# sevagh/xumx-sliCQ

Hardware: AMD Instinct MI355X
Metric: real-time factor (audio-s demixed / wall-s), 44.1 kHz stereo, offline model (higher is better)
Workload: dtype f32; 1 GPU; BASELINE configs[1]: offline model (Bark-262 sliCQT), one 240 s stereo track (10,584,000 samples, 5 chunks) per GPU, Wiener off (mix-phase), seeded synthetic weights; parallelism=one track per rank, 1 rank(s), no data-path collective

## Files before the change

xumx_slicq_amd/csrc/cdae.hip:

```cpp
#include <algorithm>
#include <cmath>
#include <cstdlib>
#include <cstring>
#include <vector>

#include "../../include/xumx_slicq_hip.h"
#include "gemm_tile.h"
#include "gemm_tile_bf3.h"
#include "gemm_tile_bf6.h"
#include "plan.h"
#include "prof.h"

#include "cdae_api.h"

namespace xsq {

__global__ __launch_bounds__(256) void k_magnitude_whiten(const float4* __restrict__ X, float4* __restrict__ xin,
                                                           const int64_t* __restrict__ cum,
                                                           const CdaeBlockDev* __restrict__ blocks,
                                                           const float* __restrict__ mean,
                                                           const float* __restrict__ scale, int nblocks,
                                                           int BC, int S, int64_t nquads, int split) {
    __shared__ int64_t cum_s[128];
    for (int i = threadIdx.x; i < nblocks && i < 128; i += 256) cum_s[i] = cum[i];
// ... 290 lines not shown
        g.in = a.act3 + (int64_t)CS * a.Bn * a.T1 * (4 * (int64_t)b.cumF1 + (int64_t)tgt * b.F1);
        g.out = nullptr;
        return g;
    }
    __device__ RowA row_a(const Group& g, int m) const {
        RowA r; r.p = nullptr; r.f = 0; r.t = 0; r.vo = BUF_OOB;
        if (m >= g.M) return r;
        int b, f, t;
        split_row(m, g.Fo, g.To, b, f, t);
        r.f = f; r.t = t;
        r.p = g.in + (((int64_t)b * g.Fi + f) * g.Ti + t) * CS;
        r.vo = 4u * (unsigned)(((b * g.Fi + f) * g.Ti + t) * CS);
        return r;
    }
    struct Cursor { int k, kk, df; };
    __device__ Cursor cursor(const Group& g, int k) const {
        Cursor c;
        c.k = k; c.df = k / (2 * CS); c.kk = k - c.df * 2 * CS;
        return c;
    }
    __device__ void advance(const Group& g, Cursor& c) const {
        c.k += 16; c.kk += 16;
        if (c.kk >= 2 * CS) { c.kk -= 2 * CS; ++c.df; }
    }
    __device__ float4 load_a4(const Group& g, const RowA& r, const Cursor& c) const { return load_at(g, r, c.k, c.df, c.kk); }
    __device__ float4 load_a4(const Group& g, const RowA& r, int k) const {
        const int df = k / (2 * CS);
        return load_at(g, r, k, df, k - df * 2 * CS);
    }
    __device__ float4 load_at(const Group& g, const RowA& r, int k, int df, int kk) const {
        const int fi = r.f - df;
        const bool pos_ok = kk < CS ? r.t >= 1 : r.t < g.Ti;
        const bool ok = k < g.K && (unsigned)fi < (unsigned)g.Fi && pos_ok;
        const unsigned vo = r.vo + 4u * (unsigned)(kk - (df * g.Ti + 1) * CS);
        return buf_ld4(buf_rsrc(g.in, 0x40000000u), ok ? vo : BUF_OOB, 0);
    }
    __device__ void epilogue(const Group& g, int row0, int n, const f32x16& a0, const f32x16& a1, bool wide) const {
        const bool v0 = n < g.N, v1 = wide && n + 32 < g.N;
        const int n1 = n + 32;
        const int ca = n >= g.hop, cb = n1 >= g.hop;
        const int dta = n - ca * g.hop, dtb = n1 - cb * g.hop;
        if (a.gx8) {
            const int64_t STp = (int64_t)g.To * g.hop, FSTp = (int64_t)g.F * STp;
            float* o = a.gx8 + 4 * (int64_t)a.Bn * g.To * g.cum + (int64_t)g.tgt * a.Bn * 2 * FSTp;
            int b, f, u;
            split_row(row0, g.Fo, g.To, b, f, u);
            int prev = 0;
#pragma unroll
            for (int r = 0; r < 16; ++r) {
                u += acc_row(r) - prev; prev = acc_row(r);
                while (u >= g.To) { u -= g.To; if (++f == g.Fo) { f = 0; ++b; } }
                if (row0 + acc_row(r) >= g.M) break;
                float* d = o + (int64_t)(b * 2) * FSTp + (int64_t)f * STp + (int64_t)u * g.hop;
                if (v0) d[ca * FSTp + dta] = a0[r];
                if (v1) d[cb * FSTp + dtb] = a1[r];
            }
            return;
        }
        const float ba = g.shift[ca], bb = g.shift[cb];
        const int FST = g.F * a.S * g.T;
        const int perb = g.Fo * g.To;
        const float2* X2 = reinterpret_cast<const float2*>(a.X) + (int64_t)a.Bn * 2 * a.S * g.cum;
        float2* Y2 = reinterpret_cast<float2*>(a.Y) + (int64_t)a.Bn * 8 * a.S * g.cum + (int64_t)g.tgt * a.Bn * 2 * FST;
        float* Mk = a.masks ? a.masks + (int64_t)a.Bn * 8 * a.S * g.cum + (int64_t)g.tgt * a.Bn * 2 * FST : nullptr;
        const int offa = ca * FST + dta, offb = cb * FST + dtb;
        const int slab0 = row0 & ~31;
        const int b0 = slab0 / perb;
        const int next_b = (b0 + 1) * perb;
        if (slab0 + 32 <= g.M && perb >= 32) {
            const int obase = row0 * g.hop + b0 * FST, ocut = next_b - row0;
            auto off = [&](int r) { return obase + acc_row(r) * g.hop + (acc_row(r) >= ocut ? FST : 0); };
            if (!a.Y && next_b >= slab0 + 32) {
                const int s0 = __builtin_amdgcn_readfirstlane(slab0);
                const int b0u = __builtin_amdgcn_readfirstlane(b0);
                const __amdgpu_buffer_rsrc_t rm = buf_rsrc(Mk + (int64_t)s0 * g.hop + (int64_t)b0u * FST, 0x40000000u);
                const unsigned lane_off = 4u * (unsigned)((row0 - slab0) * g.hop);
                const unsigned va = v0 ? lane_off + 4u * (unsigned)offa : BUF_OOB, vb = v1 ? lane_off + 4u * (unsigned)offb : BUF_OOB;
#pragma unroll
                for (int r = 0; r < 16; ++r)
                    __builtin_amdgcn_raw_buffer_store_b32(__builtin_bit_cast(unsigned, __builtin_amdgcn_rcpf(1.f + __expf(-(a0[r] + ba)))), rm, (int)va, 4 * acc_row(r) * g.hop, 0);
                if (wide) {
#pragma unroll
                    for (int r = 0; r < 16; ++r)
                        __builtin_amdgcn_raw_buffer_store_b32(__builtin_bit_cast(unsigned, __builtin_amdgcn_rcpf(1.f + __expf(-(a1[r] + bb)))), rm, (int)vb, 4 * acc_row(r) * g.hop, 0);
                }
                return;
            }
            if (!a.Y) {
                if (v0) {
#pragma unroll
                    for (int r = 0; r < 16; ++r) Mk[off(r) + offa] = __builtin_amdgcn_rcpf(1.f + __expf(-(a0[r] + ba)));
                }
                if (v1) {
#pragma unroll
                    for (int r = 0; r < 16; ++r) Mk[off(r) + offb] = __builtin_amdgcn_rcpf(1.f + __expf(-(a1[r] + bb)));
                }
                return;
            }
#pragma unroll
            for (int r0 = 0; r0 < 16; r0 += 4) {
                if (v0) {
                    float2 x[4];
#pragma unroll
                    for (int q = 0; q < 4; ++q) x[q] = X2[off(r0 + q) + offa];
#pragma unroll
                    for (int q = 0; q < 4; ++q) {
                        const float mk = __builtin_amdgcn_rcpf(1.f + __expf(-(a0[r0 + q] + ba)));
                        Y2[off(r0 + q) + offa] = make_float2(mk * x[q].x, mk * x[q].y);
                    }
                }
                if (v1) {
                    float2 x[4];
#pragma unroll
                    for (int q = 0; q < 4; ++q) x[q] = X2[off(r0 + q) + offb];
#pragma unroll
                    for (int q = 0; q < 4; ++q) {
                        const float mk = __builtin_amdgcn_rcpf(1.f + __expf(-(a1[r0 + q] + bb)));
                        Y2[off(r0 + q) + offb] = make_float2(mk * x[q].x, mk * x[q].y);
                    }
                }
            }
            if (Mk) {
                if (v0) {
#pragma unroll
                    for (int r = 0; r < 16; ++r) Mk[off(r) + offa] = __builtin_amdgcn_rcpf(1.f + __expf(-(a0[r] + ba)));
                }
                if (v1) {
#pragma unroll
                    for (int r = 0; r < 16; ++r) Mk[off(r) + offb] = __builtin_amdgcn_rcpf(1.f + __expf(-(a1[r] + bb)));
                }
            }
            return;
        }
#pragma unroll
        for (int r = 0; r < 16; ++r) {
            const int m = row0 + acc_row(r);
            if (m >= g.M) break;
            const int o = m * g.hop + (m / perb) * FST;
            if (v0) {
                const float mk = __builtin_amdgcn_rcpf(1.f + __expf(-(a0[r] + ba)));
                if (a.Y) { const float2 x = X2[o + offa]; Y2[o + offa] = make_float2(mk * x.x, mk * x.y); }
                if (Mk) Mk[o + offa] = mk;
            }
            if (v1) {
                const float mk = __builtin_amdgcn_rcpf(1.f + __expf(-(a1[r] + bb)));
                if (a.Y) { const float2 x = X2[o + offb]; Y2[o + offb] = make_float2(mk * x.x, mk * x.y); }
                if (Mk) Mk[o + offb] = mk;
            }
        }
    }
    __device__ void epilogue16(const Group& g, int rowb, int lane, int n0, const f32x4 (&acc)[2]) const {
        const int n = n0 + (lane & 15), q16 = lane >> 4;
        if (n >= g.N) return;
        const int c = n >= g.hop, dt = n - c * g.hop;
        const float bias = g.shift[c];
        const int FST = g.F * a.S * g.T, perb = g.Fo * g.To;
        const float2* X2 = reinterpret_cast<const float2*>(a.X) + (int64_t)a.Bn * 2 * a.S * g.cum;
        float2* Y2 = a.Y ? reinterpret_cast<float2*>(a.Y) + (int64_t)a.Bn * 8 * a.S * g.cum + (int64_t)g.tgt * a.Bn * 2 * FST : nullptr;
        float* Mk = a.masks ? a.masks + (int64_t)a.Bn * 8 * a.S * g.cum + (int64_t)g.tgt * a.Bn * 2 * FST : nullptr;
        const int off = c * FST + dt;
        if (!Y2 && rowb + 32 <= g.M && perb >= 32) {
            const int m0 = rowb + 4 * q16;
            const int b0 = rowb / perb;
            const int obase = m0 * g.hop + b0 * FST + off, ocut = (b0 + 1) * perb - m0;
            float mk[2][4];
#pragma unroll
            for (int rb = 0; rb < 2; ++rb)
#pragma unroll
                for (int r = 0; r < 4; ++r) mk[rb][r] = __builtin_amdgcn_rcpf(1.f + __expf(-(acc[rb][r] + bias)));
#pragma unroll
            for (int rb = 0; rb < 2; ++rb)
#pragma unroll
                for (int r = 0; r < 4; ++r) {
                    const int dm = 16 * rb + r;
                    Mk[obase + dm * g.hop + (dm >= ocut ? FST : 0)] = mk[rb][r];
                }
            return;
        }
#pragma unroll
        for (int rb = 0; rb < 2; ++rb)
#pragma unroll
            for (int r = 0; r < 4; ++r) {
                const int m = rowb + 16 * rb + 4 * q16 + r;
                if (m >= g.M) continue;
                const int o = m * g.hop + (m / perb) * FST + off;
                const float mk = __builtin_amdgcn_rcpf(1.f + __expf(-(acc[rb][r] + bias)));
                if (Y2) { const float2 x = X2[o]; Y2[o] = make_float2(mk * x.x, mk * x.y); }
                if (Mk) Mk[o] = mk;
            }
    }
};

}
#include "cdae_slab.h"
#include "cdae_wino.h"
#include "cdae_wino23.h"
#include "cdae_wino4.h"
#include "cdae_l1f.h"
#include "cdae_l4f.h"
namespace xsq {


static bool wino4_wanted() { return getenv("XSQ_WINO4") && atoi(getenv("XSQ_WINO4")) != 0; }

static int kf_of(int F) { return F < 10 ? 1 : (F < 20 ? 3 : 5); }

static int get_cdae_tiles(xsq_model* Mo, int layer, int Bn, int S, TileTable* out, bool n16 = false, bool tgt_outer = false) {
    const TileKey key{TileKind::CdaeGemm, Bn, S, layer, (n16 ? 1 : 0) | (tgt_outer ? 2 : 0)};
    return cached_tiles<TileDev>(Mo->mu, Mo->tiles, key, out, [&](std::vector<TileDev>& t) {
        const int T1 = Mo->causal ? 2 * S : 2 * S - 1, T2 = T1 - 3;
        const std::vector<int> order = order_descending(Mo->nblocks, [&](int b) {
            const CdaeBlockDev& d = Mo->blocks[b];
            return layer == 1 ? 2 * d.kf * d.T : (layer >= 4 ? d.kf * 2 * CS : d.kf * 4 * CS);
        });
        for (int b : order) {
            const CdaeBlockDev& d = Mo->blocks[b];
            int64_t M; int N;
            switch (layer) {
                case 1: M = (int64_t)Bn * d.F1 * T1; N = CS; break;
                case 2: M = (int64_t)Bn * d.F2 * T2; N = CS; break;
                case 3: M = (int64_t)Bn * d.F1 * T1; N = CS; break;
                case 4: M = (int64_t)Bn * d.F * 2 * S; N = d.T; break;
                default: M = (int64_t)Bn * d.F * (T1 + 1); N = d.T; break;
            }
            if (layer == 1 || layer == 4 || layer == 6) {
                auto push = [&](int64_t m0, int n0, int tgt) {
                    const int rem = N - n0;
                    const int kind = n16 ? (rem <= 16 ? 2 : rem <= 32 ? 1 : rem <= 48 ? 3 : 0) : (rem <= 32 ? 1 : 0);
                    t.push_back(TileDev{b * 4 + tgt, (int)m0, n0, kind});
                };
                if (tgt_outer) {
                    for (int tgt = 0; tgt < NT; ++tgt)
                        for (int64_t m0 = 0; m0 < M; m0 += 128)
                            for (int n0 = 0; n0 < N; n0 += 64) push(m0, n0, tgt);
                } else {
                    for (int64_t m0 = 0; m0 < M; m0 += 128)
                        for (int n0 = 0; n0 < N; n0 += 64)
                            for (int tgt = 0; tgt < NT; ++tgt) push(m0, n0, tgt);
                }
            } else {
                for (int tgt = 0; tgt < NT; ++tgt) push_group_tiles(t, b * 4 + tgt, M, N);
            }
        }
    });
}

static std::vector<int> blocks_by_taps(const xsq_model* Mo) {
    return order_descending(Mo->nblocks, [&](int b) { return Mo->blocks[b].kf; });
}

static int get_slab_tiles(xsq_model* Mo, int layer, int Bn, int S, TileTable* out) {
    return cached_tiles<SlabTileDev>(Mo->mu, Mo->tiles, TileKey{TileKind::CdaeSlab, Bn, S, layer, 0}, out, [&](std::vector<SlabTileDev>& t) {
        const int T1 = Mo->causal ? 2 * S : 2 * S - 1, T2 = T1 - 3;
        for (int b : blocks_by_taps(Mo)) {
            const CdaeBlockDev& d = Mo->blocks[b];
            const int64_t perb = layer == 2 ? (int64_t)d.F2 * T2 : (int64_t)d.F1 * T1;
            for (int tgt = 0; tgt < NT; ++tgt) {
                const int64_t off1 = (int64_t)CS * Bn * T1 * (4 * (int64_t)d.cumF1 + (int64_t)tgt * d.F1);
                const int64_t off2 = (int64_t)CS * Bn * T2 * (4 * (int64_t)d.cumF2 + (int64_t)tgt * d.F2);
                SlabTileDev e;
                e.kf = d.kf;
                if (layer == 2) { e.Fo = d.F2; e.Fi = d.F1; e.in_off = off1; e.out_off = off2; e.shift_off = d.s2[tgt]; e.w_off = d.w2[tgt]; }
                else { e.Fo = d.F1; e.Fi = d.F2; e.in_off = off2; e.out_off = off1; e.shift_off = d.s3[tgt]; e.w_off = d.w3[tgt]; }
                const int To = layer == 2 ? T2 : T1;
                e.pad = 0;
                for (int bi = 0; bi < Bn; ++bi)
                    for (int64_t r = 0; r < perb; r += SLAB_ROWS) {
                        e.m0 = (int)(bi * perb + r); e.b = bi; e.f0 = (int)(r / To); e.t0 = (int)(r % To);
                        t.push_back(e);
                    }
            }
        }
    });
}

static bool block_fuses23(const CdaeBlockDev& d) { return d.kf == 1 && d.F1 == d.F2; }

static int get_wino_tiles(xsq_model* Mo, int layer, int Bn, int S, TileTable* out, int outs = 2, bool skip_fused = false) {
    return cached_tiles<WinoTileDev>(Mo->mu, Mo->tiles, TileKey{TileKind::CdaeWino, Bn, S, layer, outs | (skip_fused ? 16 : 0)}, out, [&](std::vector<WinoTileDev>& t) {
        const int T1 = Mo->causal ? 2 * S : 2 * S - 1, T2 = T1 - 3;
        const int To = layer == 2 ? T2 : T1, P = (To + outs - 1) / outs, len = outs == 4 ? W4_QUADS : WN_PAIRS;
        for (int b : blocks_by_taps(Mo)) {
            const CdaeBlockDev& d = Mo->blocks[b];
            if (skip_fused && block_fuses23(d)) continue;
            for (int tgt = 0; tgt < NT; ++tgt) {
                const int64_t off1 = (int64_t)CS * Bn * T1 * (4 * (int64_t)d.cumF1 + (int64_t)tgt * d.F1);
                const int64_t off2 = (int64_t)CS * Bn * T2 * (4 * (int64_t)d.cumF2 + (int64_t)tgt * d.F2);
                WinoTileDev e;
                e.kf = d.kf; e.P = P;
                if (layer == 2) { e.Fo = d.F2; e.Fi = d.F1; e.in_off = off1; e.out_off = off2; e.shift_off = d.s2[tgt]; e.u_off = (outs == 4 ? d.uq2 : d.u2)[tgt]; }
                else { e.Fo = d.F1; e.Fi = d.F2; e.in_off = off2; e.out_off = off1; e.shift_off = d.s3[tgt]; e.u_off = (outs == 4 ? d.uq3 : d.u3)[tgt]; }
                const int perb = e.Fo * P;
                e.pad0 = e.pad1 = 0;
                for (int bi = 0; bi < Bn; ++bi)
                    for (int Q = 0; Q < perb; Q += len) {
                        e.Q0 = Q; e.b = bi;
                        t.push_back(e);
                    }
            }
        }
    });
}

static int get_wino23_tiles(xsq_model* Mo, int Bn, int S, TileTable* out) {
    return cached_tiles<Wino23TileDev>(Mo->mu, Mo->tiles, TileKey{TileKind::CdaeWino23, Bn, S, 23, 0}, out, [&](std::vector<Wino23TileDev>& t) {
        const int T1 = Mo->causal ? 2 * S : 2 * S - 1, P = (T1 + 1) / 2;
        for (int b : blocks_by_taps(Mo)) {
            const CdaeBlockDev& d = Mo->blocks[b];
            if (!block_fuses23(d)) continue;
            for (int tgt = 0; tgt < NT; ++tgt) {
                Wino23TileDev e;
                e.F = d.F1;
                e.in_off = e.out_off = (int64_t)CS * Bn * T1 * (4 * (int64_t)d.cumF1 + (int64_t)tgt * d.F1);
                e.shift2_off = d.s2[tgt]; e.shift3_off = d.s3[tgt]; e.u2_off = d.u2[tgt]; e.u3_off = d.u3[tgt];
                for (int bi = 0; bi < Bn; ++bi)
                    for (int f = 0; f < d.F1; ++f)
                        for (int A = 0; A < P; A += WN23_OUT) {
                            e.A = A; e.f = f; e.b = bi;
                            t.push_back(e);
                        }
            }
        }
    });
}

static int get_l1f_tiles(xsq_model* Mo, int Bn, int S, TileTable* out) {
    return cached_tiles<L1fTileDev>(Mo->mu, Mo->tiles, TileKey{TileKind::CdaeL1f, Bn, S, 1, 0}, out, [&](std::vector<L1fTileDev>& t) {
        const int T1 = 2 * S - 1, P = (T1 + 1) / 2;
        for (int b : order_descending(Mo->nblocks, [&](int b) { return Mo->blocks[b].nch1; })) {
            const CdaeBlockDev& d = Mo->blocks[b];
            L1fTileDev e;
            e.kf = d.kf; e.F = d.F; e.F1 = d.F1; e.hop = d.hop; e.nchunks = d.nch1; e.P = P;
            e.in_off = (int64_t)Bn * 2 * S * d.cum;
            const int total = Bn * d.F1 * P;
            e.pad0 = 0;
            for (int Q = 0; Q < total; Q += LF_PAIRS)
                for (int tgt = 0; tgt < NT; ++tgt) {
                    e.Q0 = Q;
                    e.out_off = (int64_t)CS * Bn * T1 * (4 * (int64_t)d.cumF1 + (int64_t)tgt * d.F1);
                    e.shift_off = d.s1[tgt]; e.u_off = d.u1[tgt];
                    t.push_back(e);
                }
        }
    });
}

static const int L4F_RUN = 6;
static int get_l4f_tiles(xsq_model* Mo, int Bn, int S, TileTable* out) {
    return cached_tiles<L4fTileDev>(Mo->mu, Mo->tiles, TileKey{TileKind::CdaeL4f, Bn, S, 4, 0}, out, [&](std::vector<L4fTileDev>& t) {
        const int T1 = 2 * S - 1, P = S;
        for (int b : blocks_by_taps(Mo)) {
            const CdaeBlockDev& d = Mo->blocks[b];
            const int W = d.T, cols = l4f_cols(W);
            const int64_t FST = (int64_t)d.F * S * d.T;
            L4fTileDev e;
            e.kf = d.kf; e.F = d.F; e.hop = d.hop; e.P = P; e.x_off = (int)((int64_t)Bn * 2 * S * d.cum);
            const int total = Bn * d.F * P;
            const int rtiles = (total + L4_PAIRS - 1) / L4_PAIRS;
            const int nruns = d.kf == 1 ? (rtiles + L4F_RUN - 1) / L4F_RUN : rtiles;
            for (int tgt = 0; tgt < NT; ++tgt) {
                e.in_off = (int64_t)CS * Bn * T1 * (4 * (int64_t)d.cumF1 + (int64_t)tgt * d.F1);
                e.out_off = (int64_t)Bn * 8 * S * d.cum + (int64_t)tgt * Bn * 2 * FST;
                e.bias_off = d.b4[tgt];
                for (int r = 0; r < nruns; ++r) {
                    const int t0 = (int)((int64_t)rtiles * r / nruns), t1 = (int)((int64_t)rtiles * (r + 1) / nruns);
                    for (int n0 = 0; n0 < cols; n0 += 64) {
                        e.Q0 = t0 * L4_PAIRS; e.run = t1 - t0; e.n0 = n0;
                        e.u_off = d.u4[tgt] + (int64_t)3 * CS * n0;
                        t.push_back(e);
                    }
                }
            }
        }
    });
}

}

using namespace xsq;

extern "C" {

int64_t xsq_model_num_params(int nblocks, const int32_t* F, const int32_t* T) {
    if (!F || !T || nblocks <= 0) return XSQ_ERR_ARG;
    int64_t n = 0;
    for (int b = 0; b < nblocks; ++b) {
        const int kf = kf_of(F[b]);
        n += 2 * F[b];
        n += NT * ((int64_t)H1 * 2 * kf * T[b] + 4 * H1 + (int64_t)H2 * H1 * kf * 4 + 4 * H2 +
                   (int64_t)H2 * H1 * kf * 4 + 4 * H1 + (int64_t)H1 * 2 * kf * T[b] + 2);
    }
    return n;
}

static int model_build(xsq_model** out, int nblocks, const int32_t* F, const int32_t* T, int causal,
                       const float* params, int64_t nparams, xsq_model** partial);

int xsq_model_create(xsq_model** out, int nblocks, const int32_t* F, const int32_t* T, int causal,
                     const float* params, int64_t nparams) {
    xsq_model* partial = nullptr;
    const int rc = model_build(out, nblocks, F, T, causal, params, nparams, &partial);
    if (rc != XSQ_OK && partial) xsq_model_destroy(partial);
    return rc;
}

static int model_build(xsq_model** out, int nblocks, const int32_t* F, const int32_t* T, int causal,
                       const float* params, int64_t nparams, xsq_model** partial) {
    XSQ_REQUIRE(out && F && T && params && nblocks > 0, "xsq_model_create: null argument");
    XSQ_REQUIRE(nparams == xsq_model_num_params(nblocks, F, T),
                "xsq_model_create: got %lld parameters, the block table needs %lld", (long long)nparams,
                (long long)xsq_model_num_params(nblocks, F, T));
    std::vector<BlockHost> table;
    int64_t sumFT = 0;
    for (int b = 0; b < nblocks; ++b) {
        XSQ_REQUIRE(F[b] >= 1 && T[b] >= 4 && T[b] % 4 == 0, "xsq_model_create: block %d has F=%d T=%d", b, F[b], T[b]);
        XSQ_REQUIRE(F[b] - 2 * (kf_of(F[b]) - 1) >= 1, "xsq_model_create: block with F=%d too small", F[b]);
        table.push_back(BlockHost{0, F[b], T[b], sumFT});
        sumFT += (int64_t)F[b] * T[b];
    }
    xsq_model* Mo = new xsq_model();
    *partial = Mo;
    Mo->causal = causal ? 1 : 0; Mo->nblocks = nblocks; Mo->sumFT = sumFT; Mo->table = table;
    Mo->wino4 = wino4_wanted();
    std::vector<float> pool, upool, mean, scale;
    std::vector<int64_t> cum(nblocks + 1, 0);
    std::vector<int> blockF(nblocks);
    const float* p = params;
    int cumF1 = 0, cumF2 = 0;
    int64_t cumF = 0;
    auto alloc = [&](size_t n) { size_t o = pool.size(); pool.resize(o + n, 0.f); return (int64_t)o; };
    auto bn_fold = [&](const float* bn, int C, int co, int64_t shift_off) {
        const float *bw = bn, *bb = bn + C, *rm = bn + 2 * C, *rv = bn + 3 * C;
        const double s = (double)bw[co] / std::sqrt((double)rv[co] + 1e-5);
        pool[shift_off + co] = (float)((double)bb[co] - (double)rm[co] * s);
        return s;
    };
    auto wino_weights = [&](const double (*G)[4], int ncomp, int UDF, int (*u_off)(int, int, int), int64_t wsrc, int kf) {
        const int K2 = kf * 4 * CS;
        const int64_t u = (int64_t)upool.size();
        upool.resize(upool.size() + (size_t)kf * UDF, 0.f);
        for (int df = 0; df < kf; ++df)
            for (int j = 0; j < ncomp; ++j)
                for (int col = 0; col < WN_COLS; ++col)
                    for (int ci = 0; ci < CS; ++ci) {
                        double acc = 0.0;
                        for (int dt = 0; dt < 4; ++dt)
                            acc += G[j][dt] * (double)pool[wsrc + (size_t)col * K2 + (df * 4 + dt) * CS + ci];
                        upool[u + (size_t)df * UDF + u_off(j, col, ci)] = (float)acc;
                    }
        return u;
    };
    for (int bi = 0; bi < nblocks; ++bi) {
        const BlockHost& hb = table[bi];
        CdaeBlockDev d;
        memset(&d, 0, sizeof(d));
        d.F = hb.F; d.T = hb.T; d.hop = hb.T / 2; d.kf = kf_of(hb.F);
        d.F1 = d.F - d.kf + 1; d.F2 = d.F1 - d.kf + 1;
        d.cumF1 = cumF1; d.cumF2 = cumF2; d.cum = hb.cum; d.cumF = cumF;
        d.ld1 = (int)round_up(2 * d.kf * d.T, 16); d.ld4 = (int)round_up(d.kf * 2 * CS, 16);
        cumF1 += d.F1; cumF2 += d.F2; cumF += d.F;
        cum[bi] = hb.cum; blockF[bi] = d.F;
        const int kf = d.kf, W = d.T, hop = d.hop;
        mean.insert(mean.end(), p, p + d.F); p += d.F;
        scale.insert(scale.end(), p, p + d.F); p += d.F;
        for (int t = 0; t < NT; ++t) {
            const float* w = p; p += (size_t)H1 * 2 * kf * W;
            const float* bn = p; p += 4 * H1;
            const int K1 = 2 * kf * W;
            d.w1[t] = alloc((size_t)64 * d.ld1);
            d.s1[t] = alloc(64);
            for (int co = 0; co < H1; ++co) {
                const double s = bn_fold(bn, H1, co, d.s1[t]);
                for (int k = 0; k < K1; ++k)
                    pool[d.w1[t] + (size_t)co * d.ld1 + k] = (float)((double)w[(size_t)co * K1 + k] * s);
            }
            {
                d.nch1 = l1f_chunks(kf, hop);
                const int64_t u = (int64_t)upool.size();
                upool.resize(upool.size() + (size_t)d.nch1 * LF_U16, 0.f);
                d.u1[t] = u;
                const int hq = (hop + 3) / 4;
                for (int s = 0; s < d.nch1; ++s)
                    for (int kk = 0; kk < 16; ++kk) {
                        const int e4 = 4 * s + kk / 4, seg = e4 / hq, dd = 4 * (e4 % hq) + kk % 4;
                        if (seg >= 2 * kf || dd >= hop) continue;
                        for (int co = 0; co < H1; ++co) {
                            const double w0 = pool[d.w1[t] + (size_t)co * d.ld1 + (size_t)seg * W + dd];
                            const double w1v = pool[d.w1[t] + (size_t)co * d.ld1 + (size_t)seg * W + hop + dd];
                            upool[u + l1f_u_off(s, 0, co, kk)] = (float)w0;
                            upool[u + l1f_u_off(s, 1, co, kk)] = (float)(w0 + w1v);
                            upool[u + l1f_u_off(s, 2, co, kk)] = (float)w1v;
                        }
                    }
            }
            w = p; p += (size_t)H2 * H1 * kf * 4;
            bn = p; p += 4 * H2;
            const int K2 = kf * 4 * CS;
            d.w2[t] = alloc((size_t)64 * K2);
            d.s2[t] = alloc(64);
            for (int co = 0; co < H2; ++co) {
                const double s = bn_fold(bn, H2, co, d.s2[t]);
                for (int ci = 0; ci < H1; ++ci)
                    for (int df = 0; df < kf; ++df)
                        for (int dt = 0; dt < 4; ++dt)
                            pool[d.w2[t] + (size_t)co * K2 + (df * 4 + dt) * CS + ci] =
                                (float)((double)w[(((size_t)co * H1 + ci) * kf + df) * 4 + dt] * s);
            }
            w = p; p += (size_t)H2 * H1 * kf * 4;
            bn = p; p += 4 * H1;
            d.w3[t] = alloc((size_t)64 * K2);
            d.s3[t] = alloc(64);
            for (int co = 0; co < H1; ++co) {
                const double s = bn_fold(bn, H1, co, d.s3[t]);
                for (int ci = 0; ci < H2; ++ci)
                    for (int df = 0; df < kf; ++df)
                        for (int dt = 0; dt < 4; ++dt)
                            pool[d.w3[t] + (size_t)co * K2 + (df * 4 + (3 - dt)) * CS + ci] =
                                (float)((double)w[(((size_t)ci * H1 + co) * kf + df) * 4 + dt] * s);
            }
            d.u2[t] = wino_weights(WN_G, 5, WN_UDF, wino_u_off, d.w2[t], kf);
            d.u3[t] = wino_weights(WN_G, 5, WN_UDF, wino_u_off, d.w3[t], kf);
            d.uq2[t] = Mo->wino4 ? wino_weights(W4_G, W4_NC, W4_UDF, wino4_u_off, d.w2[t], kf) : -1;
            d.uq3[t] = Mo->wino4 ? wino_weights(W4_G, W4_NC, W4_UDF, wino4_u_off, d.w3[t], kf) : -1;
            w = p; p += (size_t)H1 * 2 * kf * W;
            const float* bias = p; p += 2;
            d.w4[t] = alloc((size_t)round_up(W, 64) * d.ld4);
            d.b4[t] = alloc(64);
            pool[d.b4[t]] = bias[0]; pool[d.b4[t] + 1] = bias[1];
            for (int ci = 0; ci < H1; ++ci)
                for (int c = 0; c < 2; ++c)
                    for (int df = 0; df < kf; ++df)
                        for (int tap = 0; tap < 2; ++tap)
                            for (int dt = 0; dt < hop; ++dt)
                                pool[d.w4[t] + (size_t)(c * hop + dt) * d.ld4 + (df * 2 + (1 - tap)) * CS + ci] =
                                    w[(((size_t)ci * 2 + c) * kf + df) * W + dt + tap * hop];
            {
                const int64_t u = (int64_t)upool.size();
                const int tapf = l4f_tap_floats(W), cols = l4f_cols(W);
                upool.resize(upool.size() + (size_t)kf * tapf, 0.f);
                d.u4[t] = u;
                for (int df = 0; df < kf; ++df)
                    for (int n0 = 0; n0 < cols; n0 += 64)
                        for (int n = n0; n < std::min(cols, n0 + 64) && n < W; ++n)
                            for (int ci = 0; ci < H1; ++ci) {
                                const double wa = pool[d.w4[t] + (size_t)n * d.ld4 + (df * 2 + 1) * CS + ci];
                                const double wb = pool[d.w4[t] + (size_t)n * d.ld4 + (df * 2 + 0) * CS + ci];
                                const size_t o = (size_t)u + (size_t)df * tapf;
                                upool[o + l4f_u_off(W, n0, 0, n, ci)] = (float)wb;
                                upool[o + l4f_u_off(W, n0, 1, n, ci)] = (float)(wa + wb);
                                upool[o + l4f_u_off(W, n0, 2, n, ci)] = (float)wa;
                            }
            }
        }
        Mo->blocks.push_back(d);
    }
    cum[nblocks] = sumFT;
    Mo->sumF = cumF; Mo->sumF1 = cumF1; Mo->sumF2 = cumF2;
    if (p - params != nparams) {
        set_error("xsq_model_create: internal parameter walk mismatch");
        return XSQ_ERR_ARG;
    }
    if (int rc = upload(Mo->d_pool, pool)) return rc;
    if (int rc = upload(Mo->d_upool, upool)) return rc;
    Mo->pool_floats = (int64_t)pool.size();
    if (int rc = upload(Mo->d_mean, mean)) return rc;
    if (int rc = upload(Mo->d_scale, scale)) return rc;
    if (int rc = upload(Mo->d_blocks, Mo->blocks)) return rc;
    if (int rc = upload(Mo->d_cum, cum)) return rc;
    if (int rc = upload(Mo->d_blockF, blockF)) return rc;
    *partial = nullptr;
    *out = Mo;
    return XSQ_OK;
}

int xsq_model_set_precision(xsq_model* Mo, int mode) {
    XSQ_REQUIRE(Mo, "xsq_model_set_precision: null model");
    XSQ_REQUIRE(mode >= 0 && mode <= 2, "xsq_model_set_precision: mode %d (0 = fp32, 1 = bf16x3, 2 = bf16x6)", mode);
    if (mode == 1 && !Mo->d_pool_split) {
        XSQ_HIP(hipMalloc(&Mo->d_pool_split, (size_t)Mo->pool_floats * 4));
        hipLaunchKernelGGL(k_split_pool, dim3((unsigned)((Mo->pool_floats + 255) / 256)), dim3(256), 0, 0, Mo->d_pool,
                           Mo->d_pool_split, Mo->pool_floats);
        XSQ_HIP(hipDeviceSynchronize());
    }
    Mo->precision = mode;
    return XSQ_OK;
}

#if XSQ_WINO_STAMPS
extern "C" int xsq_debug_wn_stamps(unsigned long long* out, int reset) {
    XSQ_HIP(hipDeviceSynchronize());
    XSQ_HIP(hipMemcpyFromSymbol(out, HIP_SYMBOL(xsq::g_wn_stamps), 8 * sizeof(unsigned long long)));
    if (reset) { unsigned long long z[8] = {0}; XSQ_HIP(hipMemcpyToSymbol(HIP_SYMBOL(xsq::g_wn_stamps), z, sizeof(z))); }
    return XSQ_OK;
}
#endif
#if XSQ_WINO4_STAMPS
extern "C" int xsq_debug_w4_stamps(unsigned long long* out, int reset) {
    XSQ_HIP(hipDeviceSynchronize());
    XSQ_HIP(hipMemcpyFromSymbol(out, HIP_SYMBOL(xsq::g_w4_stamps), 8 * sizeof(unsigned long long)));
    if (reset) { unsigned long long z[8] = {0}; XSQ_HIP(hipMemcpyToSymbol(HIP_SYMBOL(xsq::g_w4_stamps), z, sizeof(z))); }
    return XSQ_OK;
}
#endif

int xsq_model_set_wiener_options(xsq_model* Mo, int softmask, int residual) {
    XSQ_REQUIRE(Mo, "xsq_model_set_wiener_options: null model");
    Mo->wiener_flags = (softmask ? XSQ_WIENER_SOFTMASK : 0) | (residual ? XSQ_WIENER_RESIDUAL : 0);
    return XSQ_OK;
}

int xsq_model_set_winograd(xsq_model* Mo, int on) {
    XSQ_REQUIRE(Mo && on >= 0 && on <= 31, "xsq_model_set_winograd: null model or mask %d (1 = layers 2 / 3 Winograd F(2, 4), 2 / 4 = layer 1 / 4 F(2, 2), 8 = F(4, 4) for long rows, "
                "16 = one-tap blocks' layers 2 and 3 in one launch)", on);
    XSQ_REQUIRE(!(on & 8) || Mo->wino4, "xsq_model_set_winograd: bit 8 (F(4, 4)) needs a model created with XSQ_WINO4=1 in the environment");
    Mo->winograd = on;
    return XSQ_OK;
}

int xsq_model_destroy(xsq_model* Mo) {
    if (!Mo) return XSQ_OK;
    for (auto& kv : Mo->tiles) (void)hipFree(kv.second.d_tiles);
    (void)hipFree(Mo->d_pool); (void)hipFree(Mo->d_upool); (void)hipFree(Mo->d_pool_split); (void)hipFree(Mo->d_mean); (void)hipFree(Mo->d_scale);
    (void)hipFree(Mo->d_blocks); (void)hipFree(Mo->d_cum); (void)hipFree(Mo->d_blockF);
// ... 209 lines not shown
```

xumx_slicq_amd/csrc/cdae_wino23.h:

```cpp
#pragma once
#include "cdae_wino.h"

namespace xsq {

constexpr int WN23_OUT = WN_PAIRS - 2;

struct Wino23TileDev {
    int A, f, F, b;
    int64_t in_off, out_off;
    int64_t shift2_off, shift3_off;
    int64_t u2_off, u3_off;
};
static_assert(sizeof(Wino23TileDev) == 64, "Wino23TileDev is meant to be one 64-byte scalar load");

template <int NV> struct Wino23Frag { float4 w[3]; float u[NV]; float wt[3]; float ut[NV]; };

__global__ __launch_bounds__(256, XSQ_WINO_WAVES_PER_EU) void cdae_wino23_kernel(CdaeArgs a, const Wino23TileDev* __restrict__ tiles, int ntiles) {
#pragma clang fp contract(off)
    constexpr int PLANE_O = WN_EROWS * WN_SLD;
    __shared__ __attribute__((aligned(16))) float slab[(WN_EROWS + WN_OROWS) * WN_SLD];
    __shared__ __attribute__((aligned(16))) float Bs[2 * 5 * WN_BTILE];

    const int tid = threadIdx.x, lane = tid & 63, wave = tid >> 6;
    const int q = lane & 15, kq = lane >> 4;
    const Wino23TileDev t = tiles[xcd_remap(blockIdx.x, ntiles)];
    asm volatile("" :: "s"(t.A), "s"(t.f), "s"(t.F), "s"(t.b), "s"(t.in_off), "s"(t.out_off), "s"(t.shift2_off), "s"(t.shift3_off),
                 "s"(t.u2_off), "s"(t.u3_off));
    const int A = t.A, f = t.f, F = t.F, b = t.b;
    const int T1 = a.T1, T2 = a.T2;

    const __amdgpu_buffer_rsrc_t ru2 = buf_rsrc(a.upool + t.u2_off, 4u * (unsigned)WN_UDF);
    const __amdgpu_buffer_rsrc_t ru3 = buf_rsrc(a.upool + t.u3_off, 4u * (unsigned)WN_UDF);
    const int b_lds0 = (tid >> 2) * WN_BLD + 4 * (tid & 3);
    float4 gb[5];
    auto load_chunk = [&](const __amdgpu_buffer_rsrc_t& ru, int s) {
        const int so = 4 * (s * WN_U16);
#pragma unroll
        for (int r = 0; r < 4; ++r) gb[r] = buf_ld4(ru, (r < 3 || tid < WN_U16 / 4 - 768) ? 16u * (unsigned)(tid + 256 * r) : BUF_OOB, so);
        if (s == 2) gb[4] = buf_ld4(ru, tid < WN_UT / 4 ? 16u * (unsigned)tid : BUF_OOB, 4 * (3 * WN_U16));
    };
    auto store_chunk = [&](int s, int buf) {
        float* Bw = Bs + buf * 5 * WN_BTILE;
#pragma unroll
        for (int r = 0; r < 4; ++r)
            *reinterpret_cast<float4*>(&Bw[(r < 3 || tid < WN_U16 / 4 - 768) ? b_lds0 + 64 * r * WN_BLD : (tid - (WN_U16 / 4 - 768)) * WN_BLD + 20]) = gb[r];
        if (s == 2) *reinterpret_cast<float4*>(&Bw[tid < WN_UT / 4 ? tid * WN_BLD + 16 : 20]) = gb[4];
    };

    constexpr int SPL = 256 / (CS / 4);
    constexpr int NPOS = 2 * WN_PAIRS + 3;
    constexpr int NLD = (NPOS + SPL - 1) / SPL;
    load_chunk(ru2, 0);
    {
        const __amdgpu_buffer_rsrc_t rin = buf_rsrc(a.act1 + t.in_off, 0x40000000u);
        const int s_p0 = tid / (CS / 4), s_c4 = tid - s_p0 * (CS / 4);
        const bool s_on = tid < SPL * (CS / 4);
        float4 sv[NLD];
#pragma unroll
        for (int r = 0; r < NLD; ++r) {
            const int j = s_p0 + SPL * r;
            const int pos = 2 * (A - 2) + j;
            const bool inr = s_on && j < NPOS && (unsigned)pos < (unsigned)T1;
            sv[r] = buf_ld4(rin, inr ? 4u * (unsigned)(((b * F + f) * T1 + pos) * CS + 4 * s_c4) : BUF_OOB, 0);
        }
#pragma unroll
        for (int r = 0; r < NLD; ++r) {
            const int j = s_p0 + SPL * r;
            if (s_on && j < NPOS) *reinterpret_cast<float4*>(&slab[((j & 1) ? PLANE_O : 0) + (j >> 1) * WN_SLD + 4 * s_c4]) = sv[r];
        }
    }
    store_chunk(0, 0);
    __syncthreads();

    const int bf = q * WN_BLD + 4 * kq;
    const int bv = 48 * WN_BLD + 4 * kq + (q & 3);
    const int pl = wave * 16 + q;
    const int eb = pl * WN_SLD + 4 * kq;
    const int ob = PLANE_O + pl * WN_SLD + 4 * kq;

    f32x4 acc[5][3];
    float accv[5][3];
    int cnt = 0;

    auto run_layer = [&](auto nv_, auto last_, const __amdgpu_buffer_rsrc_t& ru) {
        constexpr int NV = decltype(nv_)::value;
        constexpr bool last = decltype(last_)::value;
#pragma unroll
        for (int j = 0; j < 5; ++j) {
#pragma unroll
            for (int cb = 0; cb < 3; ++cb) acc[j][cb] = f32x4{0.f, 0.f, 0.f, 0.f};
#pragma unroll
            for (int cc = 0; cc < NV; ++cc) accv[j][cc] = 0.f;
        }
        auto read_frag = [&](Wino23Frag<NV>& fr, const float* Bt, bool tail) {
            fr.w[0] = *reinterpret_cast<const float4*>(&Bt[bf]);
            fr.w[1] = *reinterpret_cast<const float4*>(&Bt[bf + 16 * WN_BLD]);
            fr.w[2] = *reinterpret_cast<const float4*>(&Bt[bf + 32 * WN_BLD]);
#pragma unroll
            for (int cc = 0; cc < NV; ++cc) fr.u[cc] = Bt[bv + cc * WN_BLD];
            if (tail) {
                const int tb = q * WN_BLD + 16 + kq;
                fr.wt[0] = Bt[tb]; fr.wt[1] = Bt[tb + 16 * WN_BLD]; fr.wt[2] = Bt[tb + 32 * WN_BLD];
#pragma unroll
                for (int cc = 0; cc < NV; ++cc) fr.ut[cc] = Bt[(48 + cc) * WN_BLD + 16 + kq];
            }
        };
#pragma unroll
        for (int s = 0; s < 3; ++s) {
            const int cur = cnt & 1;
            if (s < 2) load_chunk(ru, s + 1);
            else if (!last) load_chunk(ru3, 0);
            const float* Bc = Bs + cur * 5 * WN_BTILE;
            float4 dn[5];
            dn[0] = *reinterpret_cast<const float4*>(&slab[eb + 16 * s]);
            dn[1] = *reinterpret_cast<const float4*>(&slab[ob + 16 * s]);
            dn[2] = *reinterpret_cast<const float4*>(&slab[eb + WN_SLD + 16 * s]);
            dn[3] = *reinterpret_cast<const float4*>(&slab[ob + WN_SLD + 16 * s]);
            dn[4] = *reinterpret_cast<const float4*>(&slab[eb + 2 * WN_SLD + 16 * s]);
            Wino23Frag<NV> fr[2];
            read_frag(fr[0], Bc, s == 2);
            float v[5][4], vt[5];
            {
                const float d[5][4] = {{dn[0].x, dn[0].y, dn[0].z, dn[0].w}, {dn[1].x, dn[1].y, dn[1].z, dn[1].w}, {dn[2].x, dn[2].y, dn[2].z, dn[2].w},
                                       {dn[3].x, dn[3].y, dn[3].z, dn[3].w}, {dn[4].x, dn[4].y, dn[4].z, dn[4].w}};
#pragma unroll
                for (int i = 0; i < 4; ++i) wino_bt(d[0][i], d[1][i], d[2][i], d[3][i], d[4][i], v[0][i], v[1][i], v[2][i], v[3][i], v[4][i]);
            }
            if (s == 2) {
                const int te = eb - 4 * kq + 48 + kq, to = ob - 4 * kq + 48 + kq;
                wino_bt(slab[te], slab[to], slab[te + WN_SLD], slab[to + WN_SLD], slab[te + 2 * WN_SLD], vt[0], vt[1], vt[2], vt[3], vt[4]);
            }
#pragma unroll
            for (int j = 0; j < 5; ++j) {
                const Wino23Frag<NV>& fg = fr[j & 1];
                if (j < 4) read_frag(fr[(j + 1) & 1], Bc + (j + 1) * WN_BTILE, s == 2);
                if (XSQ_WINO_SCHED2 >= 0) __builtin_amdgcn_sched_barrier(XSQ_WINO_SCHED2);
                const float wa[4] = {fg.w[0].x, fg.w[0].y, fg.w[0].z, fg.w[0].w}, wb[4] = {fg.w[1].x, fg.w[1].y, fg.w[1].z, fg.w[1].w};
                const float wc[4] = {fg.w[2].x, fg.w[2].y, fg.w[2].z, fg.w[2].w};
#pragma unroll
                for (int i = 0; i < 4; ++i) {
                    acc[j][0] = __builtin_amdgcn_mfma_f32_16x16x4f32(wa[i], v[j][i], acc[j][0], 0, 0, 0);
                    acc[j][1] = __builtin_amdgcn_mfma_f32_16x16x4f32(wb[i], v[j][i], acc[j][1], 0, 0, 0);
                    acc[j][2] = __builtin_amdgcn_mfma_f32_16x16x4f32(wc[i], v[j][i], acc[j][2], 0, 0, 0);
                }
                if (s == 2) {
                    acc[j][0] = __builtin_amdgcn_mfma_f32_16x16x4f32(fg.wt[0], vt[j], acc[j][0], 0, 0, 0);
                    acc[j][1] = __builtin_amdgcn_mfma_f32_16x16x4f32(fg.wt[1], vt[j], acc[j][1], 0, 0, 0);
                    acc[j][2] = __builtin_amdgcn_mfma_f32_16x16x4f32(fg.wt[2], vt[j], acc[j][2], 0, 0, 0);
                }
#pragma unroll
                for (int cc = 0; cc < NV; ++cc) {
                    asm("v_fmac_f32_dpp %0, %1, %2 row_newbcast:0 row_mask:0xf bank_mask:0xf\n\t"
                        "v_fmac_f32_dpp %0, %1, %3 row_newbcast:1 row_mask:0xf bank_mask:0xf\n\t"
                        "v_fmac_f32_dpp %0, %1, %4 row_newbcast:2 row_mask:0xf bank_mask:0xf\n\t"
                        "v_fmac_f32_dpp %0, %1, %5 row_newbcast:3 row_mask:0xf bank_mask:0xf"
                        : "+v"(accv[j][cc])
                        : "v"(fg.u[cc]), "v"(v[j][0]), "v"(v[j][1]), "v"(v[j][2]), "v"(v[j][3]));
                    if (s == 2) asm("v_fmac_f32 %0, %1, %2" : "+v"(accv[j][cc]) : "v"(vt[j]), "v"(fg.ut[cc]));
                }
                if (XSQ_WINO_SCHED >= 0) __builtin_amdgcn_sched_barrier(XSQ_WINO_SCHED);
            }
            if (s < 2) store_chunk(s + 1, cur ^ 1);
            else if (!last) store_chunk(0, cur ^ 1);
            cnt += 1;
            __syncthreads();
        }
    };

    auto outputs_main = [&](const float* shift, int cb, float4& o0, float4& o1) {
        const float4 sh = *reinterpret_cast<const float4*>(shift + 16 * cb + 4 * kq);
        const float shv[4] = {sh.x, sh.y, sh.z, sh.w};
        float y0[4], y1[4];
#pragma unroll
        for (int r = 0; r < 4; ++r) {
            const float m0 = acc[0][cb][r], m1 = acc[1][cb][r], m2 = acc[2][cb][r], m3 = acc[3][cb][r], m4 = acc[4][cb][r];
            y0[r] = fmaxf(((m0 + m1) + (m2 + m3)) + shv[r], 0.f);
            y1[r] = fmaxf((fmaf(2.f, m3, m1 - m2) + m4) + shv[r], 0.f);
        }
        o0 = make_float4(y0[0], y0[1], y0[2], y0[3]);
        o1 = make_float4(y1[0], y1[1], y1[2], y1[3]);
    };
    auto outputs_vec = [&](auto nv_, const float* shift, float4& o0, float4& o1) {
        constexpr int NV = decltype(nv_)::value;
        float y0v[4] = {0.f, 0.f, 0.f, 0.f}, y1v[4] = {0.f, 0.f, 0.f, 0.f};
#pragma unroll
        for (int cc = 0; cc < NV; ++cc) {
            float m[5];
#pragma unroll
            for (int j = 0; j < 5; ++j) {
                float x = accv[j][cc];
                x += __shfl_xor(x, 16);
                x += __shfl_xor(x, 32);
                m[j] = x;
            }
            y0v[cc] = ((m[0] + m[1]) + (m[2] + m[3]));
            y1v[cc] = fmaf(2.f, m[3], m[1] - m[2]) + m[4];
        }
        const float4 sh = *reinterpret_cast<const float4*>(shift + 48);
        o0 = make_float4(fmaxf(y0v[0] + sh.x, 0.f), fmaxf(y0v[1] + sh.y, 0.f), fmaxf(y0v[2] + sh.z, 0.f), fmaxf(y0v[3] + sh.w, 0.f));
        o1 = make_float4(fmaxf(y1v[0] + sh.x, 0.f), fmaxf(y1v[1] + sh.y, 0.f), fmaxf(y1v[2] + sh.z, 0.f), fmaxf(y1v[3] + sh.w, 0.f));
    };

    run_layer(std::integral_constant<int, H2 - 48>{}, std::false_type{}, ru2);
    {
        const float* shift = a.pool + t.shift2_off;
        const int t2 = 2 * (A - 2 + pl);
        const bool in0 = (unsigned)t2 < (unsigned)T2, in1 = (unsigned)(t2 + 1) < (unsigned)T2;
        auto keep = [](bool in, const float4& o) { return make_float4(in ? o.x : 0.f, in ? o.y : 0.f, in ? o.z : 0.f, in ? o.w : 0.f); };
        float* d0 = slab + PLANE_O + (pl - 1) * WN_SLD;
        float* d1 = slab + pl * WN_SLD;
#pragma unroll
        for (int cb = 0; cb < 3; ++cb) {
            float4 o0, o1;
            outputs_main(shift, cb, o0, o1);
            if (pl > 0) *reinterpret_cast<float4*>(d0 + 16 * cb + 4 * kq) = keep(in0, o0);
            *reinterpret_cast<float4*>(d1 + 16 * cb + 4 * kq) = keep(in1, o1);
        }
        float4 o0, o1;
        outputs_vec(std::integral_constant<int, H2 - 48>{}, shift, o0, o1);
        if (kq == 0) {
            if (pl > 0) *reinterpret_cast<float4*>(d0 + 48) = keep(in0, o0);
            *reinterpret_cast<float4*>(d1 + 48) = keep(in1, o1);
        }
    }
    __syncthreads();

    run_layer(std::integral_constant<int, H1 - 48>{}, std::true_type{}, ru3);
    {
        const float* shift = a.pool + t.shift3_off;
        const __amdgpu_buffer_rsrc_t ro = buf_rsrc(a.act3 + t.out_off, 0x40000000u);
        const int qq = A + pl;
        const bool ok0 = pl < WN23_OUT && 2 * qq < T1, ok1 = pl < WN23_OUT && 2 * qq + 1 < T1;
        const unsigned vo = 4u * (unsigned)((((b * F + f) * T1) + 2 * qq) * CS + 4 * kq);
#pragma unroll
        for (int cb = 0; cb < 3; ++cb) {
            float4 o0, o1;
            outputs_main(shift, cb, o0, o1);
            buf_st4(o0, ro, ok0 ? vo + 64u * cb : BUF_OOB, 0);
            buf_st4(o1, ro, ok1 ? vo + 64u * cb + 4u * CS : BUF_OOB, 0);
        }
        float4 o0, o1;
        outputs_vec(std::integral_constant<int, H1 - 48>{}, shift, o0, o1);
        const unsigned vt48 = vo - 16u * (unsigned)kq;
        buf_st4(o0, ro, (ok0 && kq == 0) ? vt48 + 192u : BUF_OOB, 0);
        buf_st4(o1, ro, (ok1 && kq == 0) ? vt48 + 192u + 4u * CS : BUF_OOB, 0);
    }
}

}
```

Measured before the change: 56030 x real-time.

## Pack two frequency rows into one Winograd-2/3 tile to fill idle lanes

Tiles of the fused layer-2/3 Winograd kernel used to cover a fixed window of output pairs within a single (batch, frequency) row, so the last tile of each row often left many positions idle. The tile generator now walks rows continuously and, when a row's tail leaves at least three spare pairs, fills them with the start of the next row. The kernel loads two input segments into the shared slab and offsets each lane's slab position and output index by its segment. This cuts the tile count and wasted compute at the cost of more complex indexing and an extra load group per tile.

```diff
diff --git a/xumx_slicq_amd/csrc/cdae.hip b/xumx_slicq_amd/csrc/cdae.hip
--- a/xumx_slicq_amd/csrc/cdae.hip
+++ b/xumx_slicq_amd/csrc/cdae.hip
@@ -616,6 +616,19 @@
     });
 }
 
+static void wino23_row_tiles(std::vector<Wino23TileDev>& t, Wino23TileDev e, int rows, int P) {
+    for (int row = 0, A = 0; row < rows;) {
+        const int c = std::min(WN23_OUT, P - A);
+        e.A = A; e.row = row; e.n0 = c + 2; e.n1 = 0;
+        A += c;
+        if (A == P) {
+            A = 0; ++row;
+            if (row < rows && WN_PAIRS - e.n0 >= 3) { e.n1 = WN_PAIRS - e.n0; A = e.n1 - 2; }
+        }
+        t.push_back(e);
+    }
+}
+
 static int get_wino23_tiles(xsq_model* Mo, int Bn, int S, TileTable* out) {
     return cached_tiles<Wino23TileDev>(Mo->mu, Mo->tiles, TileKey{TileKind::CdaeWino23, Bn, S, 23, 0}, out, [&](std::vector<Wino23TileDev>& t) {
         const int T1 = Mo->causal ? 2 * S : 2 * S - 1, P = (T1 + 1) / 2;
@@ -624,15 +637,9 @@
             if (!block_fuses23(d)) continue;
             for (int tgt = 0; tgt < NT; ++tgt) {
                 Wino23TileDev e;
-                e.F = d.F1;
                 e.in_off = e.out_off = (int64_t)CS * Bn * T1 * (4 * (int64_t)d.cumF1 + (int64_t)tgt * d.F1);
                 e.shift2_off = d.s2[tgt]; e.shift3_off = d.s3[tgt]; e.u2_off = d.u2[tgt]; e.u3_off = d.u3[tgt];
-                for (int bi = 0; bi < Bn; ++bi)
-                    for (int f = 0; f < d.F1; ++f)
-                        for (int A = 0; A < P; A += WN23_OUT) {
-                            e.A = A; e.f = f; e.b = bi;
-                            t.push_back(e);
-                        }
+                wino23_row_tiles(t, e, Bn * d.F1, P);
             }
         }
     });
diff --git a/xumx_slicq_amd/csrc/cdae_wino23.h b/xumx_slicq_amd/csrc/cdae_wino23.h
--- a/xumx_slicq_amd/csrc/cdae_wino23.h
+++ b/xumx_slicq_amd/csrc/cdae_wino23.h
@@ -6,7 +6,7 @@
 constexpr int WN23_OUT = WN_PAIRS - 2;
 
 struct Wino23TileDev {
-    int A, f, F, b;
+    int A, row, n0, n1;
     int64_t in_off, out_off;
     int64_t shift2_off, shift3_off;
     int64_t u2_off, u3_off;
@@ -24,9 +24,9 @@
     const int tid = threadIdx.x, lane = tid & 63, wave = tid >> 6;
     const int q = lane & 15, kq = lane >> 4;
     const Wino23TileDev t = tiles[xcd_remap(blockIdx.x, ntiles)];
-    asm volatile("" :: "s"(t.A), "s"(t.f), "s"(t.F), "s"(t.b), "s"(t.in_off), "s"(t.out_off), "s"(t.shift2_off), "s"(t.shift3_off),
+    asm volatile("" :: "s"(t.A), "s"(t.row), "s"(t.n0), "s"(t.n1), "s"(t.in_off), "s"(t.out_off), "s"(t.shift2_off), "s"(t.shift3_off),
                  "s"(t.u2_off), "s"(t.u3_off));
-    const int A = t.A, f = t.f, F = t.F, b = t.b;
+    const int A = t.A, row = t.row, n0 = t.n0, n1 = t.n1;
     const int T1 = a.T1, T2 = a.T2;
 
     const __amdgpu_buffer_rsrc_t ru2 = buf_rsrc(a.upool + t.u2_off, 4u * (unsigned)WN_UDF);
@@ -48,26 +48,31 @@
     };
 
     constexpr int SPL = 256 / (CS / 4);
-    constexpr int NPOS = 2 * WN_PAIRS + 3;
-    constexpr int NLD = (NPOS + SPL - 1) / SPL;
+    constexpr int NLD = (2 * WN_PAIRS + 3 + SPL - 1) / SPL;
     load_chunk(ru2, 0);
     {
-        const __amdgpu_buffer_rsrc_t rin = buf_rsrc(a.act1 + t.in_off, 0x40000000u);
-        const int s_p0 = tid / (CS / 4), s_c4 = tid - s_p0 * (CS / 4);
-        const bool s_on = tid < SPL * (CS / 4);
-        float4 sv[NLD];
-#pragma unroll
-        for (int r = 0; r < NLD; ++r) {
-            const int j = s_p0 + SPL * r;
-            const int pos = 2 * (A - 2) + j;
-            const bool inr = s_on && j < NPOS && (unsigned)pos < (unsigned)T1;
-            sv[r] = buf_ld4(rin, inr ? 4u * (unsigned)(((b * F + f) * T1 + pos) * CS + 4 * s_c4) : BUF_OOB, 0);
-        }
-#pragma unroll
-        for (int r = 0; r < NLD; ++r) {
-            const int j = s_p0 + SPL * r;
-            if (s_on && j < NPOS) *reinterpret_cast<float4*>(&slab[((j & 1) ? PLANE_O : 0) + (j >> 1) * WN_SLD + 4 * s_c4]) = sv[r];
-        }
+        const int rowb = 4 * T1 * CS;
+        const float* in0 = a.act1 + t.in_off + (int64_t)row * (T1 * CS);
+        const __amdgpu_buffer_rsrc_t rin[2] = {buf_rsrc(in0, (unsigned)rowb), buf_rsrc(in0 + T1 * CS, n1 > 0 ? (unsigned)rowb : 0u)};
+        const int len[2] = {2 * n0 + 3, n1 > 0 ? 2 * n1 + 3 : 0};
+        const int s_p0 = tid < SPL * (CS / 4) ? tid / (CS / 4) : 4 * WN_PAIRS, s_c4 = tid % (CS / 4);
+        const int par = s_p0 & 1;
+        const int jb = 4 * (s_p0 * CS + 4 * s_c4);
+        const int vb[2] = {jb + 8 * (A - 2) * CS, jb - 16 * CS};
+        const int la = (par ? PLANE_O : 0) + (s_p0 >> 1) * WN_SLD + 4 * s_c4;
+        const int lb = (par ? 0 : PLANE_O) + ((s_p0 + SPL) >> 1) * WN_SLD + 4 * s_c4;
+        const int l[2][2] = {{la, lb}, {la + (par ? n0 + 1 : n0 + 2) * WN_SLD, lb + (par ? n0 + 2 : n0 + 1) * WN_SLD}};
+        float4 sv[2][NLD];
+#pragma unroll
+        for (int g = 0; g < 2; ++g)
+#pragma unroll
+            for (int r = 0; r < NLD; ++r)
+                sv[g][r] = buf_ld4(rin[g], s_p0 + SPL * r < len[g] ? (unsigned)(vb[g] + 4 * SPL * CS * r) : BUF_OOB, 0);
+#pragma unroll
+        for (int g = 0; g < 2; ++g)
+#pragma unroll
+            for (int r = 0; r < NLD; ++r)
+                if (s_p0 + SPL * r < len[g]) *reinterpret_cast<float4*>(&slab[l[g][r & 1] + (r >> 1) * SPL * WN_SLD]) = sv[g][r];
     }
     store_chunk(0, 0);
     __syncthreads();
@@ -75,8 +80,11 @@
     const int bf = q * WN_BLD + 4 * kq;
     const int bv = 48 * WN_BLD + 4 * kq + (q & 3);
     const int pl = wave * 16 + q;
-    const int eb = pl * WN_SLD + 4 * kq;
-    const int ob = PLANE_O + pl * WN_SLD + 4 * kq;
+    const int myseg = pl >= n0 ? 1 : 0;
+    const int pi = pl - (myseg ? n0 : 0);
+    const int As = myseg ? 0 : A, ns = myseg ? n1 : n0;
+    const int eb = (pl + 2 * myseg) * WN_SLD + 4 * kq;
+    const int ob = PLANE_O + (pl + myseg) * WN_SLD + 4 * kq;
 
     f32x4 acc[5][3];
     float accv[5][3];
@@ -204,22 +212,22 @@
     run_layer(std::integral_constant<int, H2 - 48>{}, std::false_type{}, ru2);
     {
         const float* shift = a.pool + t.shift2_off;
-        const int t2 = 2 * (A - 2 + pl);
+        const int t2 = 2 * (As - 2 + pi);
         const bool in0 = (unsigned)t2 < (unsigned)T2, in1 = (unsigned)(t2 + 1) < (unsigned)T2;
         auto keep = [](bool in, const float4& o) { return make_float4(in ? o.x : 0.f, in ? o.y : 0.f, in ? o.z : 0.f, in ? o.w : 0.f); };
-        float* d0 = slab + PLANE_O + (pl - 1) * WN_SLD;
-        float* d1 = slab + pl * WN_SLD;
+        float* d0 = slab + PLANE_O + (pl + myseg - 1) * WN_SLD;
+        float* d1 = slab + (pl + 2 * myseg) * WN_SLD;
 #pragma unroll
         for (int cb = 0; cb < 3; ++cb) {
             float4 o0, o1;
             outputs_main(shift, cb, o0, o1);
-            if (pl > 0) *reinterpret_cast<float4*>(d0 + 16 * cb + 4 * kq) = keep(in0, o0);
+            if (pi > 0) *reinterpret_cast<float4*>(d0 + 16 * cb + 4 * kq) = keep(in0, o0);
             *reinterpret_cast<float4*>(d1 + 16 * cb + 4 * kq) = keep(in1, o1);
         }
         float4 o0, o1;
         outputs_vec(std::integral_constant<int, H2 - 48>{}, shift, o0, o1);
         if (kq == 0) {
-            if (pl > 0) *reinterpret_cast<float4*>(d0 + 48) = keep(in0, o0);
+            if (pi > 0) *reinterpret_cast<float4*>(d0 + 48) = keep(in0, o0);
             *reinterpret_cast<float4*>(d1 + 48) = keep(in1, o1);
         }
     }
@@ -229,9 +237,9 @@
     {
         const float* shift = a.pool + t.shift3_off;
         const __amdgpu_buffer_rsrc_t ro = buf_rsrc(a.act3 + t.out_off, 0x40000000u);
-        const int qq = A + pl;
-        const bool ok0 = pl < WN23_OUT && 2 * qq < T1, ok1 = pl < WN23_OUT && 2 * qq + 1 < T1;
-        const unsigned vo = 4u * (unsigned)((((b * F + f) * T1) + 2 * qq) * CS + 4 * kq);
+        const int qq = As + pi;
+        const bool ok0 = pi < ns - 2 && 2 * qq < T1, ok1 = pi < ns - 2 && 2 * qq + 1 < T1;
+        const unsigned vo = 4u * (unsigned)((((row + myseg) * T1) + 2 * qq) * CS + 4 * kq);
 #pragma unroll
         for (int cb = 0; cb < 3; ++cb) {
             float4 o0, o1;
```

New measurement: 56170 x real-time (median of 6 runs). No clear change (+0.3%).
